# songxf1024/GIMS

Measured on AMD Instinct MI355X. Metric: image-pairs/sec at 2x4096 keypoints, higher is better.
Workload: dtype bf16 MFMA attention + bf16x3 MFMA linears + f32 Sinkhorn; 1 GPU; 8 pairs/step/GPU of 2x4096 synthetic keypoints (kept 4096/4096 after AGC r=15 p=2 m=7), 256-d descriptors, 18 attentional layers (9 self + 9 cross), 100 Sinkhorn iterations, match_threshold 0.2; keypoints=4096

## Files before the change

gims_amd/csrc/attention.hip:

```cpp
#include "common.h"

#include <atomic>
#include <stdio.h>
#include <stdlib.h>

namespace gims {

constexpr int DH = 64;
constexpr int KB = 64;
constexpr int QW = 32;
constexpr int ATT_WAVES = 4;
constexpr int QB = QW * ATT_WAVES;
constexpr int VR_LD = 80;
typedef short s16x4 __attribute__((ext_vector_type(4)));

typedef _Float16 f16x8 __attribute__((ext_vector_type(8)));
typedef _Float16 f16x2 __attribute__((ext_vector_type(2)));
template <bool F16>
__device__ __forceinline__ f32x16 mfma_16b(bf16x8 a, bf16x8 b, f32x16 c) {
  if constexpr (F16) return __builtin_amdgcn_mfma_f32_32x32x16_f16(__builtin_bit_cast(f16x8, a), __builtin_bit_cast(f16x8, b), c, 0, 0, 0);
  else return __builtin_amdgcn_mfma_f32_32x32x16_bf16(a, b, c, 0, 0, 0);
}
template <bool F16>
__device__ __forceinline__ uint32_t pack_16b(float lo, float hi) {
// ... 235 lines not shown
#pragma unroll
      for (int i = 0; i < 2; ++i)
#pragma unroll
        for (int g = 0; g < 4; ++g) {
          const float4 v = make_float4(o[qi][i][4 * g] * inv, o[qi][i][4 * g + 1] * inv, o[qi][i][4 * g + 2] * inv, o[qi][i][4 * g + 3] * inv);
          const int col = col0 + 32 * i + 8 * g;
          if (out) *(float4*)(out + grow * ld_out + col) = v;
          if (out_hi) {
            const uint32_t h01 = pack_bf2(v.x, v.y), h23 = pack_bf2(v.z, v.w);
            const uint32_t l01 = pack_bf2(v.x - __uint_as_float(h01 << 16), v.y - __uint_as_float(h01 & 0xffff0000u));
            const uint32_t l23 = pack_bf2(v.z - __uint_as_float(h23 << 16), v.w - __uint_as_float(h23 & 0xffff0000u));
            *(uint2*)(out_hi + grow * ld_split + spl_col(col)) = make_uint2(h01, h23);
            *(uint2*)(out_lo + grow * ld_split + spl_col(col)) = make_uint2(l01, l23);
          }
        }
    }
  }
  if (stat) peak_acc_flush(pacc, stat, head);
}


constexpr int ATT8_WAVES = 8;
typedef float f32x2 __attribute__((ext_vector_type(2)));

constexpr int PS_Q = 32;
template <bool F16, int NW>
__device__ __forceinline__ void attention_peak_sample_wg(const uint16_t* __restrict__ qkv, int64_t ld, int q_col, int k_col, const gims_attn_problem pr,
                                                         int head, float c, unsigned long long* __restrict__ stat, float* xm, float* xl) {
  const int lane = threadIdx.x & 63, wave = __builtin_amdgcn_readfirstlane(threadIdx.x >> 6);
  const int li = lane & 31, lh = lane >> 5;
  const int n_s = pr.n_q < PS_Q ? pr.n_q : PS_Q;
  if (n_s <= 0 || pr.n_kv <= 0) return;
  bf16x8 qf[4];
  {
    const int j = li < n_s ? li : n_s - 1;
    const int qr = (int)(((long long)j * pr.n_q) / n_s);
    const uint16_t* qp = qkv + (int64_t)(pr.q_off + qr) * ld + q_col + head * DH + 8 * lh;
#pragma unroll
    for (int s = 0; s < 4; ++s) qf[s] = *(const bf16x8*)(qp + 16 * s);
  }
  const int n_tiles = (pr.n_kv + 31) / 32;
  float m_run = -1e30f, l_run = 0.f;
  constexpr int TB = 4;
  for (int t0 = wave; t0 < n_tiles; t0 += NW * TB) {
    bf16x8 kf[TB][4];
#pragma unroll
    for (int b = 0; b < TB; ++b) {
      const int t = t0 + b * NW;
      int kr = t * 32 + li;
      kr = kr < pr.n_kv ? kr : pr.n_kv - 1;
      const uint16_t* kp = qkv + (int64_t)(pr.kv_off + kr) * ld + k_col + head * DH + 8 * lh;
#pragma unroll
      for (int s = 0; s < 4; ++s) kf[b][s] = *(const bf16x8*)(kp + 16 * s);
    }
#pragma unroll
    for (int b = 0; b < TB; ++b) {
      const int t = t0 + b * NW;
      if (t >= n_tiles) break;
      f32x16 sacc;
#pragma unroll
      for (int r = 0; r < 16; ++r) sacc[r] = 0.f;
#pragma unroll
      for (int s = 0; s < 4; ++s) sacc = mfma_16b<F16>(kf[b][s], qf[s], sacc);
      float tmax = -1e30f;
#pragma unroll
      for (int r = 0; r < 16; ++r) {
        const int key = t * 32 + (r & 3) + 8 * (r >> 2) + 4 * lh;
        if (key >= pr.n_kv) sacc[r] = -1e30f;
        tmax = fmaxf(tmax, sacc[r]);
      }
      const float m_new = fmaxf(m_run, tmax);
      float sum = 0.f;
#pragma unroll
      for (int r = 0; r < 16; ++r) sum += __builtin_amdgcn_exp2f((sacc[r] - m_new) * c);
      l_run = l_run * __builtin_amdgcn_exp2f((m_run - m_new) * c) + sum;
      m_run = m_new;
    }
  }
  xm[wave * 64 + lane] = m_run;
  xl[wave * 64 + lane] = l_run;
  __syncthreads();
  if (wave == 0) {
    float m = -1e30f;
#pragma unroll
    for (int w = 0; w < NW; ++w) m = fmaxf(m, fmaxf(xm[w * 64 + li], xm[w * 64 + li + 32]));
    float l = 0.f;
#pragma unroll
    for (int w = 0; w < NW; ++w)
      l += xl[w * 64 + li] * __builtin_amdgcn_exp2f((xm[w * 64 + li] - m) * c) + xl[w * 64 + li + 32] * __builtin_amdgcn_exp2f((xm[w * 64 + li + 32] - m) * c);
    emit_peak_stat(stat, head, 1.f / l, lh == 0 && li < n_s);
  }
}

template <bool F16>
__device__ __forceinline__ float attention_rowmax_wave(const uint16_t* __restrict__ qkv, int64_t ld, int q_col, int k_col, const gims_attn_problem pr,
                                                       int head, float c, int qr) {
  const int lane = threadIdx.x & 63, li = lane & 31, lh = lane >> 5;
  bf16x8 qf[4];
  {
    const uint16_t* qp = qkv + (int64_t)(pr.q_off + qr) * ld + q_col + head * DH + 8 * lh;
#pragma unroll
    for (int s = 0; s < 4; ++s) qf[s] = *(const bf16x8*)(qp + 16 * s);
  }
  const int n_tiles = (pr.n_kv + 31) / 32;
  float m_run = -1e30f, l_run = 0.f;
  constexpr int TB = 2;
  for (int t0 = 0; t0 < n_tiles; t0 += TB) {
    bf16x8 kf[TB][4];
#pragma unroll
    for (int b = 0; b < TB; ++b) {
      int kr = (t0 + b) * 32 + li;
      kr = kr < pr.n_kv ? kr : pr.n_kv - 1;
      const uint16_t* kp = qkv + (int64_t)(pr.kv_off + kr) * ld + k_col + head * DH + 8 * lh;
#pragma unroll
      for (int s = 0; s < 4; ++s) kf[b][s] = *(const bf16x8*)(kp + 16 * s);
    }
#pragma unroll
    for (int b = 0; b < TB; ++b) {
      const int t = t0 + b;
      if (t >= n_tiles) break;
      f32x16 sacc;
#pragma unroll
      for (int r = 0; r < 16; ++r) sacc[r] = 0.f;
#pragma unroll
      for (int s = 0; s < 4; ++s) sacc = mfma_16b<F16>(kf[b][s], qf[s], sacc);
      float tmax = -1e30f;
#pragma unroll
      for (int r = 0; r < 16; ++r) {
        const int key = t * 32 + (r & 3) + 8 * (r >> 2) + 4 * lh;
        if (key >= pr.n_kv) sacc[r] = -1e30f;
        tmax = fmaxf(tmax, sacc[r]);
      }
      const float m_new = fmaxf(m_run, tmax);
      float sum = 0.f;
#pragma unroll
      for (int r = 0; r < 16; ++r) sum += __builtin_amdgcn_exp2f((sacc[r] - m_new) * c);
      l_run = l_run * __builtin_amdgcn_exp2f((m_run - m_new) * c) + sum;
      m_run = m_new;
    }
  }
  const float m_o = __shfl_xor(m_run, 32, 64), l_o = __shfl_xor(l_run, 32, 64);
  const float m = fmaxf(m_run, m_o);
  const float l = l_run * __builtin_amdgcn_exp2f((m_run - m) * c) + l_o * __builtin_amdgcn_exp2f((m_o - m) * c);
  return 1.f / l;
}

template <bool PROF, bool NOFMA, bool F16 = false>
__global__ __launch_bounds__(512) void attention8_bf16_kernel(
    const uint16_t* __restrict__ qkv, int64_t ld, int q_col, int k_col, int v_col,
    const gims_attn_problem* __restrict__ problems, int n_groups, int n_heads, int n_qt, float* __restrict__ out,
    int64_t ld_out, uint16_t* __restrict__ out_hi, uint16_t* __restrict__ out_lo, int64_t ld_split, unsigned long long* prof,
    int exact_only, float c, unsigned long long* __restrict__ stat, int n_sample) {
  unsigned long long pt = 0, pacc[10] = {0, 0, 0, 0, 0, 0, 0, 0, 0, 0};
  const unsigned long long t_entry = PROF ? __builtin_readcyclecounter() : 0, r_entry = PROF ? __builtin_amdgcn_s_memrealtime() : 0;
  unsigned long long t_loop0 = 0, t_loop1 = 0;
  auto stamp_work = [&](int ph) __attribute__((always_inline)) { if (PROF) { const unsigned long long n = __builtin_readcyclecounter(); pacc[2 * ph] += n - pt; pt = n; } };
  auto stamp_sub = [&](int i) __attribute__((always_inline)) {
    if (PROF) { __builtin_amdgcn_sched_barrier(0); const unsigned long long n = __builtin_readcyclecounter(); pacc[i] += n - pt; pt = n; __builtin_amdgcn_sched_barrier(0); } };
  auto stamp_wait = [&](int ph) __attribute__((always_inline)) { if (PROF) { const unsigned long long n = __builtin_readcyclecounter(); pacc[2 * ph + 1] += n - pt; pt = n; } };
  auto raw_barrier = [&]() __attribute__((always_inline)) {
    asm volatile("s_waitcnt lgkmcnt(0)" ::: "memory");
    __builtin_amdgcn_s_barrier();
    asm volatile("" ::: "memory");
  };
#define ATT8_BAR(ph) do { stamp_work(ph); raw_barrier(); stamp_wait(ph); } while (0)
  __shared__ __attribute__((aligned(16))) uint16_t Ks[2][KB * DH];
  constexpr int VROW = 96;
  __shared__ __attribute__((aligned(16))) uint16_t Vs[2][KB * VROW];
  constexpr int QP = 2, QWV = QW * QP, QBK = QWV * ATT8_WAVES;

  if (stat != nullptr && (int)blockIdx.x < n_sample) {
    if ((int)blockIdx.x < n_groups)
      attention_peak_sample_wg<F16, ATT8_WAVES>(qkv, ld, q_col, k_col, problems[blockIdx.x / n_heads], (int)blockIdx.x % n_heads, c, stat, (float*)&Ks[0][0],
                                                (float*)&Ks[1][0]);
    return;
  }
  const int bid = (int)blockIdx.x - (stat != nullptr ? n_sample : 0);
  const int xcd = bid & 7, slot = bid >> 3;
  const int group = (slot / n_qt) * 8 + xcd;
  if (group >= n_groups) return;
  const gims_attn_problem pr = problems[group / n_heads];
  const int q0 = (slot % n_qt) * QBK;
  if (q0 >= pr.n_q) return;
  const int head = group % n_heads;
  const int t = threadIdx.x, lane = t & 63;
  const int wave = __builtin_amdgcn_readfirstlane(t >> 6);
  const int li = lane & 31, lh = lane >> 5;

  uint4 rk, rv;
  const int n_tiles = (pr.n_kv + KB - 1) / KB;
  auto load_tile = [&](int kt) __attribute__((always_inline)) {
    const int kbase = kt * KB;
    const int row = t >> 3, ch = t & 7;
    int kr = kbase + row; kr = kr < pr.n_kv ? kr : pr.n_kv - 1;
    const uint16_t* base = qkv + (int64_t)pr.kv_off * ld + head * DH;
    const uint32_t off = (uint32_t)kr * (uint32_t)ld + 8u * (uint32_t)ch;
    rk = *(const uint4*)(base + k_col + off);
    rv = *(const uint4*)(base + v_col + off);
  };
  load_tile(0);
  bool tile0_requested = true;
  __shared__ __attribute__((aligned(16))) uint16_t QE[ATT8_WAVES * 32 * 132];
  static_assert(ATT8_WAVES * 32 * 132 >= 512 * DH, "the Q rows of a workgroup fit the epilogue staging array");
  bf16x8 qf[QP][4];
#pragma unroll
  for (int qi = 0; qi < QP; ++qi) {
    int qr = q0 + wave * QWV + qi * QW + li;
    qr = qr < pr.n_q ? qr : pr.n_q - 1;
    const uint16_t* qp = qkv + (int64_t)(pr.q_off + qr) * ld + q_col + head * DH + 8 * lh;
#pragma unroll
    for (int s = 0; s < 4; ++s) qf[qi][s] = *(const bf16x8*)(qp + 16 * s);
  }
  if constexpr (F16) {
#pragma unroll
    for (int qi = 0; qi < QP; ++qi)
#pragma unroll
      for (int s = 0; s < 4; ++s) *(bf16x8*)(QE + (wave * QWV) * DH + k_off(qi * QW + li, 2 * s + lh)) = qf[qi][s];
    asm volatile("s_waitcnt lgkmcnt(0)" ::: "memory");
  }
  __builtin_amdgcn_s_waitcnt(0x0F70);
  f32x16 o[QP][2];
  f32x16 nref[F16 ? QP : 1];
  constexpr float DEFER = 5.0f;
  const float defer_raw = DEFER / c;
  float m_run[QP], l_run[QP];
  float hmass[QP];

  auto store_tile = [&](int buf) __attribute__((always_inline)) {
    *(uint4*)(Ks[buf] + k_off(t >> 3, t & 7)) = rk;
    *(uint4*)(Vs[buf] + (t >> 3) * VROW + 8 * (t & 7)) = rv;
  };

  f32x16 sacc[QP][2];
  bf16x8 pf[QP][4];
  auto seg_qk = [&](int kt) __attribute__((always_inline)) {
    const int buf = kt & 1;
    if constexpr (F16) {
      bf16x8 kf[2][4], qh[QP][4];
#pragma unroll
      for (int b = 0; b < 2; ++b)
#pragma unroll
        for (int s = 0; s < 4; ++s) kf[b][s] = *(const bf16x8*)(Ks[buf] + k_off(b * 32 + li, 2 * s + lh));
#pragma unroll
      for (int qi = 0; qi < QP; ++qi)
#pragma unroll
        for (int s = 0; s < 4; ++s) qh[qi][s] = *(const bf16x8*)(QE + (wave * QWV) * DH + k_off(qi * QW + li, 2 * s + lh));
#pragma unroll
      for (int b = 0; b < 2; ++b)
#pragma unroll
        for (int s = 0; s < 4; ++s)
#pragma unroll
          for (int qi = 0; qi < QP; ++qi) sacc[qi][b] = mfma_16b<F16>(kf[b][s], qh[qi][s], s == 0 ? nref[qi] : sacc[qi][b]);
      return;
    }
#pragma unroll
    for (int qi = 0; qi < QP; ++qi)
#pragma unroll
      for (int b = 0; b < 2; ++b)
#pragma unroll
        for (int r = 0; r < 16; ++r) sacc[qi][b][r] = 0.f;
    bf16x8 kf[2][4];
#pragma unroll
    for (int b = 0; b < 2; ++b)
#pragma unroll
      for (int s = 0; s < 4; ++s) kf[b][s] = *(const bf16x8*)(Ks[buf] + k_off(b * 32 + li, 2 * s + lh));
#pragma unroll
    for (int b = 0; b < 2; ++b)
#pragma unroll
      for (int s = 0; s < 4; ++s)
#pragma unroll
        for (int qi = 0; qi < QP; ++qi) sacc[qi][b] = mfma_16b<F16>(kf[b][s], qf[qi][s], sacc[qi][b]);
    __builtin_amdgcn_sched_group_barrier(0x100, 8, 0);
    __builtin_amdgcn_sched_group_barrier(0x008, 16, 0);
  };
  auto seg_softmax = [&](int kt, int qi, bool exact) __attribute__((always_inline)) {
    const int kbase = kt * KB;
    if (kbase + KB > pr.n_kv) {
#pragma unroll
      for (int b = 0; b < 2; ++b)
#pragma unroll
        for (int r = 0; r < 16; ++r) {
          const int key = kbase + b * 32 + (r & 3) + 8 * (r >> 2) + 4 * lh;
          if (key >= pr.n_kv) sacc[qi][b][r] = -1e30f;
        }
    }
    if constexpr (F16) {
      if (!exact) {
        constexpr float RAISE = 10.f;
        float tmax = -1e30f;
#pragma unroll
        for (int b = 0; b < 2; ++b)
#pragma unroll
          for (int r = 0; r < 16; ++r) tmax = fmaxf(tmax, sacc[qi][b][r]);
        tmax = fmaxf(tmax, __shfl_xor(tmax, 32, 64));
        if (kt == 0 || __any(tmax * c > RAISE)) {
          const float dmax = kt == 0 ? tmax : fmaxf(tmax, 0.f);
          const float alpha = kt == 0 ? 1.f : __builtin_amdgcn_exp2f(-dmax * c);
          m_run[qi] += dmax;
          l_run[qi] *= alpha;
#pragma unroll
          for (int i = 0; i < 2; ++i)
#pragma unroll
            for (int r = 0; r < 16; ++r) o[qi][i][r] *= alpha;
#pragma unroll
          for (int b = 0; b < 2; ++b)
#pragma unroll
            for (int r = 0; r < 16; ++r) sacc[qi][b][r] -= dmax;
#pragma unroll
          for (int r = 0; r < 16; ++r) nref[qi][r] = -m_run[qi];
        }
        f32x2 lsum2 = {0.f, 0.f};
#pragma unroll
        for (int b = 0; b < 2; ++b) {
          float pv[16];
#pragma unroll
          for (int r = 0; r < 16; ++r) pv[r] = NOFMA ? __builtin_amdgcn_exp2f(sacc[qi][b][r]) : __builtin_amdgcn_exp2f(sacc[qi][b][r] * c);
#pragma unroll
          for (int r = 0; r < 16; r += 2) lsum2 += f32x2{pv[r], pv[r + 1]};
#pragma unroll
          for (int h2 = 0; h2 < 2; ++h2) {
            uint4 pk;
            pk.x = pack_16b<F16>(pv[8 * h2 + 0], pv[8 * h2 + 1]);
            pk.y = pack_16b<F16>(pv[8 * h2 + 2], pv[8 * h2 + 3]);
            pk.z = pack_16b<F16>(pv[8 * h2 + 4], pv[8 * h2 + 5]);
            pk.w = pack_16b<F16>(pv[8 * h2 + 6], pv[8 * h2 + 7]);
            pf[qi][2 * b + h2] = __builtin_bit_cast(bf16x8, pk);
          }
        }
        l_run[qi] += lsum2.x + lsum2.y;
        return;
      }
    }
    const bool track = exact || (!NOFMA && kt == 0);
    if (track) {
      float tmax = -1e30f;
#pragma unroll
      for (int b = 0; b < 2; ++b)
#pragma unroll
        for (int r = 0; r < 16; ++r) tmax = fmaxf(tmax, sacc[qi][b][r]);
      tmax = fmaxf(tmax, __shfl_xor(tmax, 32, 64));
      if (__any(tmax > m_run[qi] + defer_raw)) {
        const float m_new = fmaxf(m_run[qi], tmax);
        const float alpha = __builtin_amdgcn_exp2f((m_run[qi] - m_new) * c);
        m_run[qi] = m_new;
        l_run[qi] *= alpha;
#pragma unroll
        for (int i = 0; i < 2; ++i)
#pragma unroll
          for (int r = 0; r < 16; ++r) o[qi][i][r] *= alpha;
      }
    }
    const float mc = m_run[qi] * c;
    f32x2 lsum2 = {0.f, 0.f};
#pragma unroll
    for (int b = 0; b < 2; ++b) {
      float pv[16];
#pragma unroll
      for (int r = 0; r < 16; ++r)
        pv[r] = (NOFMA && !exact) ? __builtin_amdgcn_exp2f(sacc[qi][b][r]) : __builtin_amdgcn_exp2f(fmaf(sacc[qi][b][r], c, -mc));
#pragma unroll
      for (int r = 0; r < 16; r += 2) lsum2 += f32x2{pv[r], pv[r + 1]};
#pragma unroll
      for (int h2 = 0; h2 < 2; ++h2) {
        uint4 pk;
        pk.x = pack_16b<F16>(pv[8 * h2 + 0], pv[8 * h2 + 1]);
        pk.y = pack_16b<F16>(pv[8 * h2 + 2], pv[8 * h2 + 3]);
        pk.z = pack_16b<F16>(pv[8 * h2 + 4], pv[8 * h2 + 5]);
        pk.w = pack_16b<F16>(pv[8 * h2 + 6], pv[8 * h2 + 7]);
        pf[qi][2 * b + h2] = __builtin_bit_cast(bf16x8, pk);
      }
    }
    const float lsum = lsum2.x + lsum2.y;
    l_run[qi] += lsum;
    if (!F16 && !exact) hmass[qi] = fmaxf(hmass[qi], lsum);
  };
  auto seg_pv = [&](int kt) __attribute__((always_inline)) {
    const int buf = kt & 1;
    bf16x8 vf[4][2];
    const uint16_t* vb = Vs[buf] + (4 * lh + ((lane & 15) >> 2)) * VROW + 16 * ((lane >> 4) & 1) + 4 * (lane & 3);
#pragma unroll
    for (int s = 0; s < 4; ++s)
#pragma unroll
      for (int i = 0; i < 2; ++i) {
        const s16x4 v0 = __builtin_amdgcn_ds_read_tr16_b64_v4i16((s16x4 __attribute__((address_space(3)))*)(vb + 16 * s * VROW + 32 * i));
        const s16x4 v1 = __builtin_amdgcn_ds_read_tr16_b64_v4i16((s16x4 __attribute__((address_space(3)))*)(vb + (16 * s + 8) * VROW + 32 * i));
        vf[s][i] = __builtin_bit_cast(bf16x8, __builtin_shufflevector(v0, v1, 0, 1, 2, 3, 4, 5, 6, 7));
      }
#pragma unroll
    for (int s = 0; s < 4; ++s)
#pragma unroll
      for (int i = 0; i < 2; ++i)
#pragma unroll
        for (int qi = 0; qi < QP; ++qi) o[qi][i] = mfma_16b<F16>(vf[s][i], pf[qi][s], o[qi][i]);
    __builtin_amdgcn_sched_group_barrier(0x100, 16, 0);
    __builtin_amdgcn_sched_group_barrier(0x008, 16, 0);
  };

  auto pass = [&](auto ex) __attribute__((always_inline)) -> bool {
  constexpr bool exact = decltype(ex)::value;
#pragma unroll
  for (int qi = 0; qi < QP; ++qi) {
    m_run[qi] = (NOFMA && !exact && !F16) ? 0.f : -1e30f; l_run[qi] = 0.f; hmass[qi] = 0.f;
    if constexpr (F16) {
#pragma unroll
      for (int r = 0; r < 16; ++r) nref[qi][r] = 0.f;
      if (!exact) m_run[qi] = 0.f;
    }
#pragma unroll
    for (int i = 0; i < 2; ++i)
#pragma unroll
      for (int r = 0; r < 16; ++r) o[qi][i][r] = 0.f;
  }
  if (!tile0_requested) load_tile(0);
  tile0_requested = false;
  store_tile(0);
  if (1 < n_tiles) load_tile(1);
  __syncthreads();
  if (PROF) { pt = __builtin_readcyclecounter(); t_loop0 = pt; }
  for (int kt = 0; kt < n_tiles; ++kt) {
    seg_qk(kt);
    stamp_work(0);
    seg_softmax(kt, 0, exact);
    stamp_work(1);
    seg_softmax(kt, 1, exact);
    stamp_work(2);
    seg_pv(kt);
    stamp_sub(8);
    if (kt + 1 < n_tiles) store_tile((kt + 1) & 1);
    stamp_sub(9);
    if (kt + 2 < n_tiles) load_tile(kt + 2);
    ATT8_BAR(3);
  }
  if (PROF) t_loop1 = __builtin_readcyclecounter();
  bool bad = false;
#pragma unroll
  for (int qi = 0; qi < QP; ++qi) bad = bad || !(l_run[qi] < 1e30f) || (NOFMA && !(l_run[qi] > 1e-30f));
  return bad;
  };
  bool ran_exact = (exact_only & 1) != 0;
  if (!ran_exact) ran_exact = __syncthreads_or(pass(std::false_type{})) != 0;
  if (ran_exact) pass(std::true_type{});
  bool short_rows = false;
  if constexpr (!F16) {
    if (stat != nullptr) {
      unsigned fx = 0u;
#pragma unroll
      for (int qi = 0; qi < QP; ++qi) {
        const float l_tot = l_run[qi] + __shfl_xor(l_run[qi], 32, 64);
        const float h = fmaxf(hmass[qi], __shfl_xor(hmass[qi], 32, 64));
        const bool row = q0 + wave * QWV + qi * QW + li < pr.n_q;
        const float frac = ran_exact ? 1.f : fminf(h / l_tot, 1.f);
        if (row && frac >= 0.5f) { const unsigned f = (unsigned)(frac * 16777216.f + 0.5f); fx = fx > f ? fx : f; }
      }
      if (__ballot(fx != 0u) != 0ull) {
        if (ran_exact || pr.n_kv >= 512) {
#pragma unroll
          for (int o2 = 32; o2 > 0; o2 >>= 1) { const unsigned other = __shfl_xor(fx, o2, 64); fx = fx > other ? fx : other; }
          if (lane == 0) atomicMax(stat + 4 * head + 2, (unsigned long long)fx);
        } else short_rows = true;
      }
    }
  }
  if (PROF && bid == 0 && (wave == 0 || wave == 4) && lane == 0)
    for (int i = 0; i < 10; ++i) prof[(wave >> 2) * 10 + i] = pacc[i];

  const bool row_stores = out_hi && !out && out_lo == out_hi + 32;
#pragma unroll
  for (int qi = 0; qi < QP; ++qi) {
    const float l_tot = l_run[qi] + __shfl_xor(l_run[qi], 32, 64);
    const float inv = 1.f / l_tot;
    const int qr = q0 + wave * QWV + qi * QW + li;
    if (row_stores) {
      uint16_t* es = QE + wave * (32 * 132);
#pragma unroll
      for (int i = 0; i < 2; ++i)
#pragma unroll
        for (int g = 0; g < 4; ++g) {
          const float4 v = make_float4(o[qi][i][4 * g] * inv, o[qi][i][4 * g + 1] * inv, o[qi][i][4 * g + 2] * inv, o[qi][i][4 * g + 3] * inv);
          const uint32_t h01 = pack_bf2(v.x, v.y), h23 = pack_bf2(v.z, v.w);
          const uint32_t l01 = pack_bf2(v.x - __uint_as_float(h01 << 16), v.y - __uint_as_float(h01 & 0xffff0000u));
          const uint32_t l23 = pack_bf2(v.z - __uint_as_float(h23 << 16), v.w - __uint_as_float(h23 & 0xffff0000u));
          uint16_t* e = es + li * 132 + 64 * i + 8 * g + 4 * lh;
          *(uint2*)e = make_uint2(h01, h23);
          *(uint2*)(e + 32) = make_uint2(l01, l23);
        }
      asm volatile("s_waitcnt lgkmcnt(0)" ::: "memory");
      const int c = lane & 15, rs = lane >> 4;
#pragma unroll
      for (int it = 0; it < 8; ++it) {
        const int r = 4 * it + rs;
        const uint4 w = *(const uint4*)(es + r * 132 + 8 * c);
        const int qrow = q0 + wave * QWV + qi * QW + r;
        if (qrow < pr.n_q) *(uint4*)(out_hi + (int64_t)(pr.q_off + qrow) * ld_split + spl_col(head * DH) + 8 * c) = w;
      }
      asm volatile("s_waitcnt lgkmcnt(0)" ::: "memory");
    } else if (qr < pr.n_q) {
      const int64_t grow = pr.q_off + qr;
      const int col0 = head * DH + 4 * lh;
#pragma unroll
      for (int i = 0; i < 2; ++i)
#pragma unroll
        for (int g = 0; g < 4; ++g) {
          const float4 v = make_float4(o[qi][i][4 * g] * inv, o[qi][i][4 * g + 1] * inv, o[qi][i][4 * g + 2] * inv, o[qi][i][4 * g + 3] * inv);
          const int col = col0 + 32 * i + 8 * g;
          if (out) *(float4*)(out + grow * ld_out + col) = v;
          if (out_hi) {
            const uint32_t h01 = pack_bf2(v.x, v.y), h23 = pack_bf2(v.z, v.w);
            const uint32_t l01 = pack_bf2(v.x - __uint_as_float(h01 << 16), v.y - __uint_as_float(h01 & 0xffff0000u));
            const uint32_t l23 = pack_bf2(v.z - __uint_as_float(h23 << 16), v.w - __uint_as_float(h23 & 0xffff0000u));
            *(uint2*)(out_hi + grow * ld_split + spl_col(col)) = make_uint2(h01, h23);
            *(uint2*)(out_lo + grow * ld_split + spl_col(col)) = make_uint2(l01, l23);
          }
        }
    }
  }
  if constexpr (!F16) {
    if (short_rows) {
      unsigned fx = 0u;
#pragma unroll 1
      for (int qi = 0; qi < QP; ++qi) {
        const int qr = q0 + wave * QWV + qi * QW + li;
        const float pmax = attention_rowmax_wave<F16>(qkv, ld, q_col, k_col, pr, head, c, qr < pr.n_q ? qr : pr.n_q - 1);
        if (qr < pr.n_q && pmax >= 0.5f) { const unsigned f = (unsigned)(fminf(pmax, 1.f) * 16777216.f + 0.5f); fx = fx > f ? fx : f; }
      }
      if (__ballot(fx != 0u) != 0ull) {
#pragma unroll
        for (int o2 = 32; o2 > 0; o2 >>= 1) { const unsigned other = __shfl_xor(fx, o2, 64); fx = fx > other ? fx : other; }
        if (lane == 0) atomicMax(stat + 4 * head + 2, (unsigned long long)fx);
      }
    }
  }
  if (PROF && bid == 0 && wave == 0 && lane == 0) {
    const unsigned long long t_exit = __builtin_readcyclecounter(), r_exit = __builtin_amdgcn_s_memrealtime();
    prof[20] = t_loop0 - t_entry; prof[21] = t_loop1 - t_loop0; prof[22] = t_exit - t_loop1; prof[23] = r_exit - r_entry;
  }
}

constexpr int X3W_VR = VR_LD;
constexpr int X3_LDS_BYTES = 2 * 2 * (KB * DH + KB * X3W_VR) * 2;

__device__ __forceinline__ void attention_x3_block(
    const uint16_t* __restrict__ qkv, int64_t ld, int q_col, int k_col, int v_col,
    const gims_attn_problem* __restrict__ problems, int n_groups, int n_heads, int n_qt, float* __restrict__ out,
    int64_t ld_out, uint16_t* __restrict__ out_hi, uint16_t* __restrict__ out_lo, int64_t ld_split, float c,
    unsigned long long* __restrict__ stat, const int bid) {
  extern __shared__ __attribute__((aligned(16))) uint16_t x3_lds[];
  auto Ks = [&](int p, int buf) __attribute__((always_inline)) { return x3_lds + (p * 2 + buf) * (KB * DH); };
  auto Vr = [&](int p, int buf) __attribute__((always_inline)) { return x3_lds + 4 * (KB * DH) + (p * 2 + buf) * (KB * X3W_VR); };

  const int xcd = bid & 7, slot = bid >> 3;
  const int group = (slot / n_qt) * 8 + xcd;
  if (group >= n_groups) return;
  const gims_attn_problem pr = problems[group / n_heads];
  const int q0 = (slot % n_qt) * QB;
  if (q0 >= pr.n_q) return;
  const int head = group % n_heads;
  const int t = threadIdx.x, lane = t & 63, wave = t >> 6;
  const int li = lane & 31, lh = lane >> 5;
  const int qs = spl_col(q_col + head * DH), ks = spl_col(k_col + head * DH), vs = spl_col(v_col + head * DH);
  auto doff = [&](int d8) __attribute__((always_inline)) { return ((d8 >> 2) << 6) + ((d8 & 3) << 3); };

  bf16x8 qh[4], ql[4];
  {
    int qr = q0 + wave * QW + li;
    qr = qr < pr.n_q ? qr : pr.n_q - 1;
    const uint16_t* qp = qkv + (int64_t)(pr.q_off + qr) * ld + qs;
#pragma unroll
    for (int s = 0; s < 4; ++s) {
      qh[s] = *(const bf16x8*)(qp + doff(2 * s + lh));
      ql[s] = *(const bf16x8*)(qp + doff(2 * s + lh) + 32);
    }
  }
  f32x16 o[2];
#pragma unroll
  for (int i = 0; i < 2; ++i)
#pragma unroll
    for (int r = 0; r < 16; ++r) o[i][r] = 0.f;
  constexpr float DEFER = 5.0f;
  const float defer_raw = DEFER / c;
  float m_run = -1e30f, l_run = 0.f, m_true = -1e30f;

  const int n_tiles = (pr.n_kv + KB - 1) / KB;
  const int wave_u = __builtin_amdgcn_readfirstlane(wave);
  auto dma_k = [&](int kt, int buf) __attribute__((always_inline)) {
    const int kbase = kt * KB;
#pragma unroll
    for (int j2 = 0; j2 < 2; ++j2) {
      const int j = wave_u * 2 + j2, row = 8 * j + (lane >> 3), ch = (lane & 7) ^ ((row >> 1) & 7);
      int kr = kbase + row; kr = kr < pr.n_kv ? kr : pr.n_kv - 1;
      const uint16_t* src = qkv + (int64_t)(pr.kv_off + kr) * ld + ks + doff(ch);
#pragma unroll
      for (int p = 0; p < 2; ++p)
        __builtin_amdgcn_global_load_lds((const __attribute__((address_space(1))) void*)(src + 32 * p),
                                         (__attribute__((address_space(3))) void*)(Ks(p, buf) + j * 512), 16, 0, 0);
    }
  };
  auto dma_v = [&](int kt, int buf) __attribute__((always_inline)) {
    const int kbase = kt * KB;
#pragma unroll
    for (int j3 = 0; j3 < 3; ++j3) {
      const int j = wave_u + 4 * j3;
      if (j < 10) {
        const int B = 1024 * j + 16 * lane, row = B / (2 * X3W_VR), pos = (B % (2 * X3W_VR)) >> 4, ch = pos < 8 ? pos : 0;
        int kr = kbase + row; kr = kr < pr.n_kv ? kr : pr.n_kv - 1;
        const uint16_t* src = qkv + (int64_t)(pr.kv_off + kr) * ld + vs + doff(ch);
#pragma unroll
        for (int p = 0; p < 2; ++p)
          __builtin_amdgcn_global_load_lds((const __attribute__((address_space(1))) void*)(src + 32 * p),
                                           (__attribute__((address_space(3))) void*)(Vr(p, buf) + j * 512), 16, 0, 0);
      }
    }
  };
  dma_k(0, 0);
  dma_v(0, 0);
  asm volatile("s_waitcnt vmcnt(0)" ::: "memory");
  __syncthreads();

  for (int kt = 0; kt < n_tiles; ++kt) {
    const int buf = kt & 1;
    if (kt + 1 < n_tiles) { dma_k(kt + 1, buf ^ 1); dma_v(kt + 1, buf ^ 1); }
    f32x16 sacc[2];
#pragma unroll
    for (int b = 0; b < 2; ++b)
#pragma unroll
      for (int r = 0; r < 16; ++r) sacc[b][r] = 0.f;
#pragma unroll
    for (int b = 0; b < 2; ++b)
#pragma unroll
      for (int s = 0; s < 4; ++s) {
        const bf16x8 kh = *(const bf16x8*)(Ks(0, buf) + k_off(b * 32 + li, 2 * s + lh));
        const bf16x8 kl = *(const bf16x8*)(Ks(1, buf) + k_off(b * 32 + li, 2 * s + lh));
        sacc[b] = __builtin_amdgcn_mfma_f32_32x32x16_bf16(kl, qh[s], sacc[b], 0, 0, 0);
        sacc[b] = __builtin_amdgcn_mfma_f32_32x32x16_bf16(kh, ql[s], sacc[b], 0, 0, 0);
        sacc[b] = __builtin_amdgcn_mfma_f32_32x32x16_bf16(kh, qh[s], sacc[b], 0, 0, 0);
      }
    const int kbase = kt * KB;
    if (kbase + KB > pr.n_kv) {
#pragma unroll
      for (int b = 0; b < 2; ++b)
#pragma unroll
        for (int r = 0; r < 16; ++r) {
          const int key = kbase + b * 32 + (r & 3) + 8 * (r >> 2) + 4 * lh;
          if (key >= pr.n_kv) sacc[b][r] = -1e30f;
        }
    }
    float tmax = -1e30f;
#pragma unroll
    for (int b = 0; b < 2; ++b)
#pragma unroll
      for (int r = 0; r < 16; ++r) tmax = fmaxf(tmax, sacc[b][r]);
    tmax = fmaxf(tmax, __shfl_xor(tmax, 32, 64));
    m_true = fmaxf(m_true, tmax);
    if (__any(tmax > m_run + defer_raw)) {
      const float m_new = fmaxf(m_run, tmax);
      const float alpha = __builtin_amdgcn_exp2f((m_run - m_new) * c);
      m_run = m_new;
      l_run *= alpha;
#pragma unroll
      for (int i = 0; i < 2; ++i)
#pragma unroll
        for (int r = 0; r < 16; ++r) o[i][r] *= alpha;
    }
    const float mc = m_run * c;
    bf16x8 ph[4], pl[4];
    float lsum = 0.f;
#pragma unroll
    for (int b = 0; b < 2; ++b) {
      float pv[16];
#pragma unroll
      for (int r = 0; r < 16; ++r) {
        pv[r] = __builtin_amdgcn_exp2f(fmaf(sacc[b][r], c, -mc));
        lsum += pv[r];
      }
#pragma unroll
      for (int h2 = 0; h2 < 2; ++h2) {
        uint32_t hw[4], lw[4];
#pragma unroll
        for (int j = 0; j < 4; ++j) {
          const float x = pv[8 * h2 + 2 * j], y = pv[8 * h2 + 2 * j + 1];
          hw[j] = pack_bf2(x, y);
          lw[j] = pack_bf2(x - __uint_as_float(hw[j] << 16), y - __uint_as_float(hw[j] & 0xffff0000u));
        }
        ph[2 * b + h2] = __builtin_bit_cast(bf16x8, make_uint4(hw[0], hw[1], hw[2], hw[3]));
        pl[2 * b + h2] = __builtin_bit_cast(bf16x8, make_uint4(lw[0], lw[1], lw[2], lw[3]));
      }
    }
    l_run += lsum;
#pragma unroll
// ... 445 lines not shown
  float* xo = (float*)sp_lds;
  if (half > 0) {
    float* dst = xo + (((half - 1) * 4 + wave) * 35) * 64 + lane;
#pragma unroll
    for (int i = 0; i < 2; ++i)
#pragma unroll
      for (int r = 0; r < 16; ++r) dst[(i * 16 + r) * 64] = o[i][r];
    dst[32 * 64] = m_run;
    dst[33 * 64] = l_run;
    dst[34 * 64] = m_true;
  }
  __syncthreads();
  if (half > 0) return;
#pragma unroll
  for (int pt = 1; pt < NS; ++pt) {
    const float* src = xo + (((pt - 1) * 4 + wave) * 35) * 64 + lane;
    const float m1 = src[32 * 64], l1 = src[33 * 64];
    m_true = fmaxf(m_true, src[34 * 64]);
    const float m_new = fmaxf(m_run, m1);
    const float a0 = __builtin_amdgcn_exp2f((m_run - m_new) * c), a1 = __builtin_amdgcn_exp2f((m1 - m_new) * c);
    m_run = m_new;
    l_run = l_run * a0 + l1 * a1;
#pragma unroll
    for (int i = 0; i < 2; ++i)
#pragma unroll
      for (int r = 0; r < 16; ++r) o[i][r] = o[i][r] * a0 + src[(i * 16 + r) * 64] * a1;
  }
  const float l_tot = l_run + __shfl_xor(l_run, 32, 64);
  const float inv = 1.f / l_tot;
  const int qr = q0 + wave * QW + li;
  if (stat) peak_acc_add(pacc, __builtin_amdgcn_exp2f((m_true - m_run) * c) * inv, lh == 0 && qr < pr.n_q);
  if (qr < pr.n_q) {
    const int64_t grow = pr.q_off + qr;
    const int col0 = head * DH + 4 * lh;
#pragma unroll
    for (int i = 0; i < 2; ++i)
#pragma unroll
      for (int g = 0; g < 4; ++g) {
        const float4 v = make_float4(o[i][4 * g] * inv, o[i][4 * g + 1] * inv, o[i][4 * g + 2] * inv, o[i][4 * g + 3] * inv);
        const int col = col0 + 32 * i + 8 * g;
        if (out) *(float4*)(out + grow * ld_out + col) = v;
        if (out_hi) {
          const uint32_t h01 = pack_bf2(v.x, v.y), h23 = pack_bf2(v.z, v.w);
          const uint32_t l01 = pack_bf2(v.x - __uint_as_float(h01 << 16), v.y - __uint_as_float(h01 & 0xffff0000u));
          const uint32_t l23 = pack_bf2(v.z - __uint_as_float(h23 << 16), v.w - __uint_as_float(h23 & 0xffff0000u));
          *(uint2*)(out_hi + grow * ld_split + spl_col(col)) = make_uint2(h01, h23);
          *(uint2*)(out_lo + grow * ld_split + spl_col(col)) = make_uint2(l01, l23);
        }
      }
  }
  if (stat) peak_acc_flush(pacc, stat, head);
}
template <int NS> constexpr int SPLIT_LDS_BYTES = NS * 2 * (KB * DH + KB * VR_LD) * 2;
static_assert(SPLIT_LDS_BYTES<2> >= 1 * 4 * 35 * 64 * 4 && SPLIT_LDS_BYTES<4> >= 3 * 4 * 35 * 64 * 4, "merge exchange must fit the staging buffers");

}

namespace gims {
__global__ __launch_bounds__(256) void attention_range_kernel(const uint16_t* __restrict__ qkv, int64_t ld, int q_col, int k_col, int v_col,
                                                              const gims_attn_problem* __restrict__ problems, int n_heads, int kind,
                                                              unsigned long long* __restrict__ stat) {
  const gims_attn_problem pr = problems[blockIdx.y];
  const int width = n_heads * DH;
  const int cpr = width / 8;
  float mx[3] = {0.f, 0.f, 0.f};
  auto fold = [&](int which, uint4 w) __attribute__((always_inline)) {
    const uint32_t u[4] = {w.x, w.y, w.z, w.w};
#pragma unroll
    for (int e = 0; e < 4; ++e) {
      float a, b;
      if (kind == 1) {
        const f16x2 h = __builtin_bit_cast(f16x2, u[e]);
        a = fabsf((float)h[0]); b = fabsf((float)h[1]);
      } else {
        a = fabsf(__uint_as_float(u[e] << 16)); b = fabsf(__uint_as_float(u[e] & 0xffff0000u));
      }
      mx[which] = fmaxf(mx[which], fmaxf(a, b));
    }
  };
#pragma unroll
  for (int which = 0; which < 3; ++which) {
    const int rows = which == 0 ? pr.n_q : pr.n_kv, off = which == 0 ? pr.q_off : pr.kv_off, col = which == 0 ? q_col : (which == 1 ? k_col : v_col);
    const int total = rows * cpr, stride = gridDim.x * blockDim.x;
    auto src = [&](int i) __attribute__((always_inline)) {
      const int r = i / cpr, ch = col + 8 * (i - r * cpr);
      return (const uint4*)(qkv + (int64_t)(off + r) * ld + (kind == 2 ? spl_col(ch) : ch));
    };
    int i = blockIdx.x * blockDim.x + threadIdx.x;
    for (; i + 3 * stride < total; i += 4 * stride) {
      const uint4 w0 = *src(i), w1 = *src(i + stride), w2 = *src(i + 2 * stride), w3 = *src(i + 3 * stride);
      fold(which, w0); fold(which, w1); fold(which, w2); fold(which, w3);
    }
    for (; i < total; i += stride) fold(which, *src(i));
  }
  __shared__ float red[3][4];
#pragma unroll
  for (int which = 0; which < 3; ++which) {
    const float m = wave_max(mx[which]);
    if ((threadIdx.x & 63) == 0) red[which][threadIdx.x >> 6] = m;
  }
  __syncthreads();
  if (threadIdx.x < 3) {
    const float m = fmaxf(fmaxf(red[threadIdx.x][0], red[threadIdx.x][1]), fmaxf(red[threadIdx.x][2], red[threadIdx.x][3]));
    unsigned long long* dst = stat + 4 * n_heads + threadIdx.x;
    if (m > 0.f && (unsigned long long)__float_as_uint(m) > __hip_atomic_load(dst, __ATOMIC_RELAXED, __HIP_MEMORY_SCOPE_AGENT)) atomicMax(dst, (unsigned long long)__float_as_uint(m));
  }
}
static int attention_range_launch(const uint16_t* qkv, int64_t ld, int q_col, int k_col, int v_col, const gims_attn_problem* problems, int n_problems,
                                  int n_heads, int kind, unsigned long long* stat, hipStream_t stream) {
  hipLaunchKernelGGL(attention_range_kernel, dim3(32, n_problems), dim3(256), 0, stream, qkv, ld, q_col, k_col, v_col, problems, n_heads, kind, stat);
  GIMS_LAUNCH_CHECK();
  return GIMS_OK;
}

static std::atomic<uint64_t> g_launch_counts[GIMS_ATTN_KERNEL_KINDS];
static inline void count_launch(int kind) { g_launch_counts[kind].fetch_add(1, std::memory_order_relaxed); }

struct AttnPrefix {
  const uint16_t* qkv; int64_t ld; int q_col, k_col, v_col; const gims_attn_problem* problems; int n_groups, n_heads;
  float* out; int64_t ld_out; uint16_t* out_hi; uint16_t* out_lo; int64_t ld_split;
  int max_n_q, groups8;
  hipStream_t stream;
};
template <typename K, typename... Tail>
static int attn_launch(K kernel, const AttnPrefix& p, int n_qt, int grid, int block, int lds, Tail... tail) {
  if (lds) GIMS_LDS_ATTR((const void*)kernel, lds);
  hipLaunchKernelGGL(kernel, dim3(grid), dim3(block), lds, p.stream, p.qkv, p.ld, p.q_col, p.k_col, p.v_col, p.problems, p.n_groups, p.n_heads, n_qt,
                     p.out, p.ld_out, p.out_hi, p.out_lo, p.ld_split, tail...);
  GIMS_LAUNCH_CHECK();
  return GIMS_OK;
}

enum class Attn16 { SPLIT2, SPLIT4, WAVE8, WAVE4_QP2, WAVE4_QP1 };
static Attn16 attn16_choose(int groups8, int max_n_q, int force, int ns_env) {
  const bool two = force == 2 || (force != 1 && groups8 * cdiv(max_n_q, 2 * QB) >= 512);
  const bool eight = force == 8 || (force == 0 && groups8 * cdiv(max_n_q, 512) >= 256);
  const int wgs = groups8 * cdiv(max_n_q, QB);
  const bool split = force == 3 || (force == 0 && !eight && !two && wgs <= 512 && max_n_q >= 512);
  if (split) return ns_env == 4 || (ns_env != 2 && wgs <= 256 && max_n_q >= 2048) ? Attn16::SPLIT4 : Attn16::SPLIT2;
  if (eight) return Attn16::WAVE8;
  return two ? Attn16::WAVE4_QP2 : Attn16::WAVE4_QP1;
}

enum class AttnX3 { NARROW, WIDE, WIDE_WALK };
static AttnX3 attn_x3_choose(int groups8, int max_n_q, int wide_env, int round, bool walk) {
  const int n_blocks = groups8 * cdiv(max_n_q, 2 * QB);
  const bool wide = wide_env < 0 ? n_blocks >= 512 : wide_env != 0;
  if (!wide) return AttnX3::NARROW;
  return walk && n_blocks > round ? AttnX3::WIDE_WALK : AttnX3::WIDE;
}

template <bool PROF, bool F16>
static int attention8_launch(const AttnPrefix& p, bool prescaled, unsigned long long* dprof, int exact_only, float c, unsigned long long* stat, int n_sample) {
  const int n_qt = cdiv(p.max_n_q, 512), grid = n_sample + p.groups8 * n_qt;
  return prescaled ? attn_launch(attention8_bf16_kernel<PROF, true, F16>, p, n_qt, grid, 512, 0, dprof, exact_only, c, stat, n_sample)
                   : attn_launch(attention8_bf16_kernel<PROF, false, F16>, p, n_qt, grid, 512, 0, dprof, exact_only, c, stat, n_sample);
}

template <bool F16>
static int attention_16b_launch(const AttnPrefix& p, bool prescaled, float c, unsigned long long* stat) {
  const Attn16 kind = attn16_choose(p.groups8, p.max_n_q, env_int("GIMS_ATTN_QP", 0), env_int("GIMS_ATTN_SPLIT", 0));
  const int n_qt = cdiv(p.max_n_q, QB), n_qt2 = cdiv(p.max_n_q, 2 * QB);
  switch (kind) {
    case Attn16::SPLIT4:
      count_launch(GIMS_ATTN_KERNEL_SPLIT);
      return attn_launch(attention_split_kernel<4, F16>, p, n_qt, p.groups8 * n_qt, 1024, SPLIT_LDS_BYTES<4>, c, stat);
    case Attn16::SPLIT2:
      count_launch(GIMS_ATTN_KERNEL_SPLIT);
      return attn_launch(attention_split_kernel<2, F16>, p, n_qt, p.groups8 * n_qt, 512, SPLIT_LDS_BYTES<2>, c, stat);
    case Attn16::WAVE4_QP2:
      count_launch(GIMS_ATTN_KERNEL_WAVE4);
      return attn_launch(attention_bf16_kernel<2, F16>, p, n_qt2, p.groups8 * n_qt2, 256, 0, c, stat);
    case Attn16::WAVE4_QP1:
      count_launch(GIMS_ATTN_KERNEL_WAVE4);
      return attn_launch(attention_bf16_kernel<1, F16>, p, n_qt, p.groups8 * n_qt, 256, 0, c, stat);
    case Attn16::WAVE8: break;
  }
  count_launch(F16 ? GIMS_ATTN_KERNEL_WAVE8_F16 : GIMS_ATTN_KERNEL_WAVE8);
  const int exact_only = env_int("GIMS_ATTN_EXACT", 0);
  static const int prof = env_int("GIMS_ATTN_PROF", 0);
  if (!prof) {
    return attention8_launch<false, F16>(p, prescaled, nullptr, exact_only, c, stat, stat ? p.groups8 : 0);
  }
  unsigned long long* dprof = (unsigned long long*)device_once("attention8_prof", 24 * sizeof(unsigned long long), nullptr);
  GIMS_CHECK_ARG(dprof, "gims_attention: no profile buffer");
  const int rc = attention8_launch<true, F16>(p, prescaled, dprof, exact_only, c, nullptr, 0);
  if (rc != GIMS_OK) return rc;
  GIMS_HIP(hipStreamSynchronize(p.stream));
  unsigned long long h[24];
  GIMS_HIP(hipMemcpy(h, dprof, sizeof(h), hipMemcpyDeviceToHost));
  fprintf(stderr, "[attention8 wave 0 of workgroup 0] prologue %llu, tile loop %llu, epilogue %llu shader cycles; %.1f us on the 100-MHz counter -> %.2f GHz\n",
          h[20], h[21], h[22], h[23] / 100.0, (double)(h[20] + h[21] + h[22]) / (h[23] / 100.0) * 1e-3);
  for (int g = 0; g < 2; ++g)
    fprintf(stderr, "[attention8 wave %d] cycles over the whole tile loop: QK %llu, softmax0 %llu, softmax1 %llu, PV %llu, store_tile %llu, "
            "load_tile %llu, barrier wait %llu\n", 4 * g, h[g * 10 + 0], h[g * 10 + 2], h[g * 10 + 4], h[g * 10 + 8], h[g * 10 + 9], h[g * 10 + 6],
            h[g * 10 + 7]);
  return GIMS_OK;
}

static int attention_x3_launch(const AttnPrefix& p, float c, unsigned long long* stat, const gims_attn_guard& guard) {
  const int round = 2 * (device_cus() & ~7);
  const AttnX3 kind = attn_x3_choose(p.groups8, p.max_n_q, env_int("GIMS_ATTN_X3W", -1), round, guard.stat && guard_walk_enabled());
  count_launch(guard.stat ? GIMS_ATTN_KERNEL_X3_GUARDED : GIMS_ATTN_KERNEL_X3);
  if (kind == AttnX3::NARROW) {
    const int n_qt = cdiv(p.max_n_q, QB), n_blocks = p.groups8 * n_qt;
    return attn_launch(attention_x3_kernel, p, n_qt, guard.stat && n_blocks > round ? round : n_blocks, 256, X3_LDS_BYTES, c, stat, guard, n_blocks);
  }
  const int n_qt = cdiv(p.max_n_q, 2 * QB), n_blocks = p.groups8 * n_qt;
  if (kind == AttnX3::WIDE_WALK) return attn_launch(attention_x3w_kernel<2, true>, p, n_qt, round, 256, X3W_LDS_BYTES, c, stat, guard, n_blocks);
  return attn_launch(attention_x3w_kernel<2, false>, p, n_qt, n_blocks, 256, X3W_LDS_BYTES, c, stat, guard, n_blocks);
}
}

extern "C" int gims_attention_launch_counts(uint64_t* counts, int32_t n, int32_t reset) {
  GIMS_CHECK_ARG(counts || n == 0, "gims_attention_launch_counts: null pointer");
  for (int i = 0; i < n && i < GIMS_ATTN_KERNEL_KINDS; ++i) counts[i] = gims::g_launch_counts[i].load(std::memory_order_relaxed);
  for (int i = GIMS_ATTN_KERNEL_KINDS; i < n; ++i) counts[i] = 0;
  if (reset) for (auto& c : gims::g_launch_counts) c.store(0, std::memory_order_relaxed);
  return GIMS_OK;
}

extern "C" int gims_attention(const gims_attn_args* args, void* stream) {
  GIMS_CHECK_ARG(args, "gims_attention: null arguments");
  const uint16_t* qkv = args->qkv;
  const int64_t ld = args->ld, ld_out = args->ld_out, ld_split = args->ld_split;
  const int32_t q_col = args->q_col, k_col = args->k_col, v_col = args->v_col, n_problems = args->n_problems, max_n_q = args->max_n_q, n_heads = args->n_heads,
                flags = args->flags;
  const gims_attn_problem* problems = args->problems;
  float* out = args->out;
  uint16_t* out_hi = args->out_hi;
  uint16_t* out_lo = args->out_lo;
  uint64_t* stat_u64 = args->stat;
  const gims_attn_guard guard = args->guard;
  GIMS_CHECK_ARG(!guard.stat || ((flags & GIMS_ATTN_X3) && !stat_u64 && (guard.kind == GIMS_GUARD_PEAKED || guard.kind == GIMS_GUARD_RANGE) &&
                                 guard.n_heads > 0 && guard.n_heads <= 15 && (((uintptr_t)guard.stat) & 7) == 0),
                 "gims_attention: a guard goes with GIMS_ATTN_X3, without a statistic of its own, kind GIMS_GUARD_*, 8-byte aligned stat");
  using namespace gims;
  GIMS_CHECK_ARG((((uintptr_t)stat_u64) & 7) == 0, "gims_attention: stat must be 8-byte aligned");
  unsigned long long* stat = (unsigned long long*)stat_u64;
  GIMS_CHECK_ARG(qkv && problems && (out || out_hi), "gims_attention: null pointer");
  GIMS_CHECK_ARG((out_hi == nullptr) == (out_lo == nullptr) && (ld_split % 8) == 0 && (((uintptr_t)out_hi | (uintptr_t)out_lo) & 15) == 0,
                 "gims_attention: out_hi/out_lo come together, 16-byte aligned, ld_split %% 8 == 0");
  GIMS_CHECK_ARG(n_problems > 0 && max_n_q > 0 && n_heads > 0, "gims_attention: empty launch");
  GIMS_CHECK_ARG((ld % 8) == 0 && (q_col % 8) == 0 && (k_col % 8) == 0 && (v_col % 8) == 0,
                 "gims_attention: qkv ld / column offsets must be multiples of 8 (16-byte loads)");
  GIMS_CHECK_ARG((ld_out % 4) == 0, "gims_attention: ld_out must be a multiple of 4");
  GIMS_CHECK_ARG(ld <= 16384, "gims_attention: qkv pitch %lld too large (32-bit tile offsets)", (long long)ld);
  const int n_groups = n_heads * n_problems;
  const AttnPrefix p = {qkv, ld, q_col, k_col, v_col, problems, n_groups, n_heads, out, ld_out, out_hi, out_lo, ld_split, max_n_q, 8 * cdiv(n_groups, 8), (hipStream_t)stream};
  const bool prescaled = (flags & GIMS_ATTN_Q_PRESCALED) != 0;
  const float c = prescaled ? 1.f : 0.125f * 1.4426950408889634f;
  const bool f16 = (flags & GIMS_ATTN_F16) != 0;
  GIMS_CHECK_ARG(!(f16 && (flags & GIMS_ATTN_X3)), "gims_attention: GIMS_ATTN_F16 and GIMS_ATTN_X3 exclude each other");
  if (stat && (flags & (GIMS_ATTN_X3 | GIMS_ATTN_F16)) && !(flags & GIMS_ATTN_NO_RANGE)) {
    const int rc = attention_range_launch(qkv, ld, q_col, k_col, v_col, problems, n_problems, n_heads, (flags & GIMS_ATTN_X3) ? 2 : (f16 ? 1 : 0), stat, p.stream);
    if (rc != GIMS_OK) return rc;
  }
  if (flags & GIMS_ATTN_X3) {
    GIMS_CHECK_ARG((q_col % 32) == 0 && (k_col % 32) == 0 && (v_col % 32) == 0 && (ld % 64) == 0,
                   "gims_attention: GIMS_ATTN_X3 takes logical column offsets that are multiples of 32 and an SPL32 pitch (multiple of 64)");
    return attention_x3_launch(p, c, stat, guard);
  }
  return f16 ? attention_16b_launch<true>(p, prescaled, c, stat) : attention_16b_launch<false>(p, prescaled, c, stat);
}
```

Before: 550.0 pairs/s.

## Make attention8 kernel persistent and prefetch next block's Q and K/V during epilogue

```diff
diff --git a/gims_amd/csrc/attention.hip b/gims_amd/csrc/attention.hip
--- a/gims_amd/csrc/attention.hip
+++ b/gims_amd/csrc/attention.hip
@@ -411,7 +411,7 @@
     int64_t ld_out, uint16_t* __restrict__ out_hi, uint16_t* __restrict__ out_lo, int64_t ld_split, unsigned long long* prof,
     int exact_only, float c, unsigned long long* __restrict__ stat, int n_sample) {
   unsigned long long pt = 0, pacc[10] = {0, 0, 0, 0, 0, 0, 0, 0, 0, 0};
-  const unsigned long long t_entry = PROF ? __builtin_readcyclecounter() : 0, r_entry = PROF ? __builtin_amdgcn_s_memrealtime() : 0;
+  unsigned long long t_entry = PROF ? __builtin_readcyclecounter() : 0, r_entry = PROF ? __builtin_amdgcn_s_memrealtime() : 0;
   unsigned long long t_loop0 = 0, t_loop1 = 0;
   auto stamp_work = [&](int ph) __attribute__((always_inline)) { if (PROF) { const unsigned long long n = __builtin_readcyclecounter(); pacc[2 * ph] += n - pt; pt = n; } };
   auto stamp_sub = [&](int i) __attribute__((always_inline)) {
@@ -428,56 +428,72 @@
   __shared__ __attribute__((aligned(16))) uint16_t Vs[2][KB * VROW];
   constexpr int QP = 2, QWV = QW * QP, QBK = QWV * ATT8_WAVES;
 
-  if (stat != nullptr && (int)blockIdx.x < n_sample) {
-    if ((int)blockIdx.x < n_groups)
-      attention_peak_sample_wg<F16, ATT8_WAVES>(qkv, ld, q_col, k_col, problems[blockIdx.x / n_heads], (int)blockIdx.x % n_heads, c, stat, (float*)&Ks[0][0],
-                                                (float*)&Ks[1][0]);
-    return;
-  }
-  const int bid = (int)blockIdx.x - (stat != nullptr ? n_sample : 0);
-  const int xcd = bid & 7, slot = bid >> 3;
-  const int group = (slot / n_qt) * 8 + xcd;
-  if (group >= n_groups) return;
-  const gims_attn_problem pr = problems[group / n_heads];
-  const int q0 = (slot % n_qt) * QBK;
-  if (q0 >= pr.n_q) return;
-  const int head = group % n_heads;
-  const int t = threadIdx.x, lane = t & 63;
-  const int wave = __builtin_amdgcn_readfirstlane(t >> 6);
-  const int li = lane & 31, lh = lane >> 5;
+  const int wave = __builtin_amdgcn_readfirstlane((int)threadIdx.x >> 6);
+  const int n_blocks = ((n_groups + 7) & ~7) * n_qt, G = (int)gridDim.x;
+  auto decode = [&](int b, gims_attn_problem& p, int& q0_, int& head_) __attribute__((always_inline)) -> bool {
+    const int xcd = b & 7, slot = b >> 3;
+    const int group = (slot / n_qt) * 8 + xcd;
+    if (group >= n_groups) return false;
+    p = problems[group / n_heads];
+    q0_ = (slot % n_qt) * QBK;
+    head_ = group % n_heads;
+    return q0_ < p.n_q;
+  };
+  auto next_block = [&](int b, gims_attn_problem& p, int& q0_, int& head_) __attribute__((always_inline)) -> int {
+    while (b < n_blocks && !decode(b, p, q0_, head_)) b += G;
+    return b;
+  };
+  auto thread_id = [&]() __attribute__((always_inline)) { int v = (int)threadIdx.x; asm volatile("" : "+v"(v)); return v; };
 
   uint4 rk, rv;
-  const int n_tiles = (pr.n_kv + KB - 1) / KB;
-  auto load_tile = [&](int kt) __attribute__((always_inline)) {
+  auto load_tile = [&](const gims_attn_problem& p, int hd, int kt, int t) __attribute__((always_inline)) {
     const int kbase = kt * KB;
     const int row = t >> 3, ch = t & 7;
-    int kr = kbase + row; kr = kr < pr.n_kv ? kr : pr.n_kv - 1;
-    const uint16_t* base = qkv + (int64_t)pr.kv_off * ld + head * DH;
+    int kr = kbase + row; kr = kr < p.n_kv ? kr : p.n_kv - 1;
+    const uint16_t* base = qkv + (int64_t)p.kv_off * ld + hd * DH;
     const uint32_t off = (uint32_t)kr * (uint32_t)ld + 8u * (uint32_t)ch;
     rk = *(const uint4*)(base + k_col + off);
     rv = *(const uint4*)(base + v_col + off);
   };
-  load_tile(0);
-  bool tile0_requested = true;
   __shared__ __attribute__((aligned(16))) uint16_t QE[ATT8_WAVES * 32 * 132];
   static_assert(ATT8_WAVES * 32 * 132 >= 512 * DH, "the Q rows of a workgroup fit the epilogue staging array");
   bf16x8 qf[QP][4];
-#pragma unroll
-  for (int qi = 0; qi < QP; ++qi) {
-    int qr = q0 + wave * QWV + qi * QW + li;
-    qr = qr < pr.n_q ? qr : pr.n_q - 1;
-    const uint16_t* qp = qkv + (int64_t)(pr.q_off + qr) * ld + q_col + head * DH + 8 * lh;
-#pragma unroll
-    for (int s = 0; s < 4; ++s) qf[qi][s] = *(const bf16x8*)(qp + 16 * s);
-  }
+  auto load_q = [&](const gims_attn_problem& p, int q0_, int hd, int t) __attribute__((always_inline)) {
+#pragma unroll
+    for (int qi = 0; qi < QP; ++qi) {
+      int qr = q0_ + wave * QWV + qi * QW + (t & 31);
+      qr = qr < p.n_q ? qr : p.n_q - 1;
+      const uint16_t* qp = qkv + (int64_t)(p.q_off + qr) * ld + q_col + hd * DH + 8 * ((t & 63) >> 5);
+#pragma unroll
+      for (int s = 0; s < 4; ++s) qf[qi][s] = *(const bf16x8*)(qp + 16 * s);
+    }
+  };
+  gims_attn_problem pr;
+  int q0 = 0, head = 0;
+  int bid = next_block((int)blockIdx.x, pr, q0, head);
+  for (bool first_block = true; bid < n_blocks; first_block = false) {
+  if (PROF && !first_block) { t_entry = __builtin_readcyclecounter(); r_entry = __builtin_amdgcn_s_memrealtime(); }
+  const int t = thread_id(), lane = t & 63, li = lane & 31, lh = lane >> 5;
+  if (!first_block) decode(bid, pr, q0, head);
+  if (first_block) {
+    load_tile(pr, head, 0, t);
+    load_q(pr, q0, head, t);
+  }
+  const int n_tiles = (pr.n_kv + KB - 1) / KB;
+  bool tile0_requested = true;
   if constexpr (F16) {
+    if (!first_block) raw_barrier();
 #pragma unroll
     for (int qi = 0; qi < QP; ++qi)
 #pragma unroll
       for (int s = 0; s < 4; ++s) *(bf16x8*)(QE + (wave * QWV) * DH + k_off(qi * QW + li, 2 * s + lh)) = qf[qi][s];
     asm volatile("s_waitcnt lgkmcnt(0)" ::: "memory");
-  }
-  __builtin_amdgcn_s_waitcnt(0x0F70);
+  } else {
+#pragma unroll
+    for (int qi = 0; qi < QP; ++qi)
+#pragma unroll
+      for (int s = 0; s < 4; ++s) asm volatile("" : "+v"(qf[qi][s]));
+  }
   f32x16 o[QP][2];
   f32x16 nref[F16 ? QP : 1];
   constexpr float DEFER = 5.0f;
@@ -670,11 +686,11 @@
 #pragma unroll
       for (int r = 0; r < 16; ++r) o[qi][i][r] = 0.f;
   }
-  if (!tile0_requested) load_tile(0);
+  if (!tile0_requested) load_tile(pr, head, 0, t);
   tile0_requested = false;
   store_tile(0);
-  if (1 < n_tiles) load_tile(1);
-  __syncthreads();
+  if (1 < n_tiles) load_tile(pr, head, 1, t);
+  raw_barrier();
   if (PROF) { pt = __builtin_readcyclecounter(); t_loop0 = pt; }
   for (int kt = 0; kt < n_tiles; ++kt) {
     seg_qk(kt);
@@ -687,7 +703,7 @@
     stamp_sub(8);
     if (kt + 1 < n_tiles) store_tile((kt + 1) & 1);
     stamp_sub(9);
-    if (kt + 2 < n_tiles) load_tile(kt + 2);
+    if (kt + 2 < n_tiles) load_tile(pr, head, kt + 2, t);
     ATT8_BAR(3);
   }
   if (PROF) t_loop1 = __builtin_readcyclecounter();
@@ -699,6 +715,23 @@
   bool ran_exact = (exact_only & 1) != 0;
   if (!ran_exact) ran_exact = __syncthreads_or(pass(std::false_type{})) != 0;
   if (ran_exact) pass(std::true_type{});
+  {
+  const int t = thread_id(), lane = t & 63, li = lane & 31, lh = lane >> 5;
+  int bid_next;
+  {
+    gims_attn_problem pr_next;
+    int q0_next, head_next;
+    bid_next = next_block(bid + G, pr_next, q0_next, head_next);
+    if (bid_next < n_blocks) {
+      load_tile(pr_next, head_next, 0, t);
+      load_q(pr_next, q0_next, head_next, t);
+    } else if constexpr (F16) {
+#pragma unroll
+      for (int qi = 0; qi < QP; ++qi)
+#pragma unroll
+        for (int s = 0; s < 4; ++s) qf[qi][s] = bf16x8{};
+    }
+  }
   bool short_rows = false;
   if constexpr (!F16) {
     if (stat != nullptr) {
@@ -789,10 +822,19 @@
       }
     }
   }
-  if (PROF && bid == 0 && wave == 0 && lane == 0) {
+  if (PROF && blockIdx.x == 0 && wave == 0 && lane == 0) {
     const unsigned long long t_exit = __builtin_readcyclecounter(), r_exit = __builtin_amdgcn_s_memrealtime();
-    prof[20] = t_loop0 - t_entry; prof[21] = t_loop1 - t_loop0; prof[22] = t_exit - t_loop1; prof[23] = r_exit - r_entry;
-  }
+    unsigned long long* span = prof + (first_block ? 20 : 24);
+    span[0] = t_loop0 - t_entry; span[1] = t_loop1 - t_loop0; span[2] = t_exit - t_loop1; span[3] = r_exit - r_entry;
+  }
+  bid = bid_next;
+  }
+  }
+  if (stat != nullptr && n_sample > 0)
+    for (int g = ((G >> 3) - 1 - ((int)blockIdx.x >> 3)) * 8 + ((int)blockIdx.x & 7); g < n_groups; g += G) {
+      __syncthreads();
+      attention_peak_sample_wg<F16, ATT8_WAVES>(qkv, ld, q_col, k_col, problems[g / n_heads], g % n_heads, c, stat, (float*)&Ks[0][0], (float*)&Ks[1][0]);
+    }
 }
 
 constexpr int X3W_VR = VR_LD;
@@ -1544,7 +1586,9 @@
 
 template <bool PROF, bool F16>
 static int attention8_launch(const AttnPrefix& p, bool prescaled, unsigned long long* dprof, int exact_only, float c, unsigned long long* stat, int n_sample) {
-  const int n_qt = cdiv(p.max_n_q, 512), grid = n_sample + p.groups8 * n_qt;
+  const int n_qt = cdiv(p.max_n_q, 512), n_blocks = p.groups8 * n_qt, cap = env_int("GIMS_ATTN8_WGS", 0);
+  int grid = std::min(n_blocks, device_cus() & ~7);
+  if (cap >= 8 && cap % 8 == 0) grid = std::min(grid, cap);
   return prescaled ? attn_launch(attention8_bf16_kernel<PROF, true, F16>, p, n_qt, grid, 512, 0, dprof, exact_only, c, stat, n_sample)
                    : attn_launch(attention8_bf16_kernel<PROF, false, F16>, p, n_qt, grid, 512, 0, dprof, exact_only, c, stat, n_sample);
 }
@@ -1574,15 +1618,20 @@
   if (!prof) {
     return attention8_launch<false, F16>(p, prescaled, nullptr, exact_only, c, stat, stat ? p.groups8 : 0);
   }
-  unsigned long long* dprof = (unsigned long long*)device_once("attention8_prof", 24 * sizeof(unsigned long long), nullptr);
+  unsigned long long* dprof = (unsigned long long*)device_once("attention8_prof", 28 * sizeof(unsigned long long), nullptr);
   GIMS_CHECK_ARG(dprof, "gims_attention: no profile buffer");
+  GIMS_HIP(hipMemsetAsync(dprof, 0, 28 * sizeof(unsigned long long), p.stream));
   const int rc = attention8_launch<true, F16>(p, prescaled, dprof, exact_only, c, nullptr, 0);
   if (rc != GIMS_OK) return rc;
   GIMS_HIP(hipStreamSynchronize(p.stream));
-  unsigned long long h[24];
+  unsigned long long h[28];
   GIMS_HIP(hipMemcpy(h, dprof, sizeof(h), hipMemcpyDeviceToHost));
-  fprintf(stderr, "[attention8 wave 0 of workgroup 0] prologue %llu, tile loop %llu, epilogue %llu shader cycles; %.1f us on the 100-MHz counter -> %.2f GHz\n",
-          h[20], h[21], h[22], h[23] / 100.0, (double)(h[20] + h[21] + h[22]) / (h[23] / 100.0) * 1e-3);
+  for (int b = 0; b < 2; ++b) {
+    const unsigned long long* s = h + 20 + 4 * b;
+    if (s[3] == 0) continue;
+    fprintf(stderr, "[attention8 wave 0 of workgroup 0, %s block] prologue %llu, tile loop %llu, epilogue %llu shader cycles; %.1f us on the 100-MHz "
+            "counter -> %.2f GHz\n", b ? "last" : "first", s[0], s[1], s[2], s[3] / 100.0, (double)(s[0] + s[1] + s[2]) / (s[3] / 100.0) * 1e-3);
+  }
   for (int g = 0; g < 2; ++g)
     fprintf(stderr, "[attention8 wave %d] cycles over the whole tile loop: QK %llu, softmax0 %llu, softmax1 %llu, PV %llu, store_tile %llu, "
             "load_tile %llu, barrier wait %llu\n", 4 * g, h[g * 10 + 0], h[g * 10 + 2], h[g * 10 + 4], h[g * 10 + 8], h[g * 10 + 9], h[g * 10 + 6],
```

Result: no change. 549.7 pairs/s (-0.1%).
